# davxy/ark-ec-vrfs

Measured on AMD Instinct MI355X. Metric: Bandersnatch IETF-ECVRF verifies/sec, 2^20 batch per GPU, higher is better.
Workload: dtype u32; 1 GPU; IETF ECVRF verify, Bandersnatch_SHA-512_ELL2, batch 2^20 per GPU, compressed points (161 B/verify), checked decode: on curve + prime-order subgroup, as arkworks' deserialisation, ad="", about 1 in 16 proofs forged (BASELINE.json configs[2]); global_batch=1048576, parallelism=items sharded x1, result gather only, subgroup_check=True

## Files before the change

### ark_ec_vrfs_amd/csrc/fe.cuh

```cuda
#pragma once
#include <hip/hip_runtime.h>
#include <cstdint>
#include "field.h"
#include "vrf_types.h"

VRF_NS_BEGIN

using vrfk::LMASK;
constexpr int NL = 9;
constexpr int LW = 29;

constexpr int mul_v(int v1, int v2) {
  return vrfk::FIELD_KIND == 2 ? 2 : 1 + (v1 * v2 * vrfk::MULV_NUM + 99999) / 100000;
}

template <int L, int V>
struct Fe {
  static_assert(L >= 1 && L <= 7, "limb bound out of range");
  static_assert(V >= 1 && V <= vrfk::VMAX, "value bound out of range (top limb must stay < 2^29)");
  uint32_t v[NL];
  Fe() = default;
  template <int L2, int V2>
  VRF_HD Fe(const Fe<L2, V2>& o) {
    static_assert(L2 <= L && V2 <= V, "narrowing Fe conversion");
#pragma unroll
    for (int i = 0; i < NL; ++i) v[i] = o.v[i];
  }
};

using FeN = Fe<1, 2>;
using FeP = Fe<1, 5>;

template <int L, int V>
VRF_HD Fe<L, V> fe_load(const uint32_t* p) {
  Fe<L, V> r;
#pragma unroll
  for (int i = 0; i < NL; ++i) r.v[i] = p[i];
  return r;
}
VRF_HD FeN fe_const(const uint32_t (&c)[NL]) {
  FeN r;
#pragma unroll
  for (int i = 0; i < NL; ++i) r.v[i] = c[i];
  return r;
}
template <int L, int V>
VRF_HD void fe_store(uint32_t* p, const Fe<L, V>& a) {
#pragma unroll
  for (int i = 0; i < NL; ++i) p[i] = a.v[i];
}

VRF_HD FeN fe_zero() {
  FeN r;
#pragma unroll
  for (int i = 0; i < NL; ++i) r.v[i] = 0;
  return r;
}
VRF_HD FeN fe_one() { return fe_const(vrfk::ONE_M); }

template <int L1, int V1, int L2, int V2>
VRF_HD Fe<L1 + L2, V1 + V2> fe_add(const Fe<L1, V1>& a, const Fe<L2, V2>& b) {
  Fe<L1 + L2, V1 + V2> r;
#pragma unroll
  for (int i = 0; i < NL; ++i) r.v[i] = a.v[i] + b.v[i];
  return r;
}

template <int K, int LB>
struct Bias;
#define VRF_BIAS(K_, LB_)                                            \
  template <>                                                        \
  struct Bias<K_, LB_> {                                             \
    static VRF_HD uint32_t at(int i) { return vrfk::BIAS_L##LB_##_K##K_[i]; } \
  };
VRF_BIAS(4, 1) VRF_BIAS(8, 1) VRF_BIAS(16, 1) VRF_BIAS(32, 1) VRF_BIAS(64, 1)
VRF_BIAS(4, 2) VRF_BIAS(8, 2) VRF_BIAS(16, 2) VRF_BIAS(32, 2) VRF_BIAS(64, 2)
#undef VRF_BIAS

constexpr int bias_k(int v) { return v < 4 ? 4 : v < 8 ? 8 : v < 16 ? 16 : v < 32 ? 32 : 64; }

template <int L1, int V1, int L2, int V2>
VRF_HD Fe<L1 + L2 + 1, V1 + bias_k(V2)> fe_sub(const Fe<L1, V1>& a, const Fe<L2, V2>& b) {
  static_assert(L2 <= 2, "subtrahend must have L <= 2 (normalise first)");
  constexpr int K = bias_k(V2);
  Fe<L1 + L2 + 1, V1 + K> r;
#pragma unroll
  for (int i = 0; i < NL; ++i) r.v[i] = a.v[i] + (Bias<K, L2>::at(i) - b.v[i]);
  return r;
}

template <int L, int V>
VRF_HD Fe<L + 1, bias_k(V)> fe_neg(const Fe<L, V>& b) {
  static_assert(L <= 2, "fe_neg operand must have L <= 2");
  constexpr int K = bias_k(V);
  Fe<L + 1, K> r;
#pragma unroll
  for (int i = 0; i < NL; ++i) r.v[i] = Bias<K, L>::at(i) - b.v[i];
  return r;
}

template <int L, int V>
VRF_HD Fe<2 * L, 2 * V> fe_dbl(const Fe<L, V>& a) {
  Fe<2 * L, 2 * V> r;
#pragma unroll
  for (int i = 0; i < NL; ++i) r.v[i] = a.v[i] << 1;
  return r;
}
template <int L, int V>
VRF_HD Fe<5 * L, 5 * V> fe_mul5(const Fe<L, V>& a) {
  Fe<5 * L, 5 * V> r;
#pragma unroll
  for (int i = 0; i < NL; ++i) r.v[i] = (a.v[i] << 2) + a.v[i];
  return r;
}

template <int L, int V>
VRF_HD Fe<1, V> fe_norm(const Fe<L, V>& a) {
  Fe<1, V> r;
  r.v[0] = a.v[0] & LMASK;
#pragma unroll
  for (int i = 1; i < NL - 1; ++i) r.v[i] = (a.v[i] & LMASK) + (a.v[i - 1] >> LW);
  r.v[NL - 1] = a.v[NL - 1] + (a.v[NL - 2] >> LW);
  return r;
}

#if VRF_FIELD == 3
template <int L, int V>
VRF_HD Fe<1, 2> fe_wred(const Fe<L, V>& a) {
  uint32_t x[NL];
  uint32_t c = 0;
#pragma unroll
  for (int i = 0; i < NL - 1; ++i) {
    const uint32_t t = a.v[i] + c;
    x[i] = t & LMASK;
    c = t >> LW;
  }
  x[NL - 1] = a.v[NL - 1] + c;
  const int32_t k = (int32_t)(x[NL - 1] >> 24);
  x[NL - 1] &= 0x00ffffffu;
  Fe<1, 2> r;
  int32_t cc = k;
#pragma unroll
  for (int i = 0; i < NL; ++i) {
    int32_t t = (int32_t)x[i] + cc;
    if (i == 3) t -= k << 9;
    if (i == 6) t -= k << 18;
    if (i == 7) t += k << 21;
    r.v[i] = (i < NL - 1) ? ((uint32_t)t & LMASK) : (uint32_t)t;
    cc = t >> LW;
  }
  return r;
}
#endif

template <int L, int V>
VRF_HD Fe<L, V> fe_select(bool c, const Fe<L, V>& a, const Fe<L, V>& b) {
  Fe<L, V> r;
#pragma unroll
  for (int i = 0; i < NL; ++i) r.v[i] = c ? a.v[i] : b.v[i];
  return r;
}

VRF_HD uint64_t mad(uint32_t a, uint32_t b, uint64_t c) { return (uint64_t)a * b + c; }
VRF_HD constexpr uint64_t mont_bias() { return vrfk::FIELD_KIND == 0 ? (uint64_t)LMASK : 0; }
VRF_HD uint32_t mont_digit(uint32_t col) {
  if constexpr (vrfk::FIELD_KIND == 0) return ~col & LMASK;
  else return (col * vrfk::NINV29) & LMASK;
}
constexpr uint32_t PM_FOLD = 1216;
constexpr int PM_TOPBITS = 23;

template <int V>
VRF_HD void pm_fold(Fe<1, V>& r, const uint32_t (&d)[2 * NL]) {
  uint64_t acc = 0;
#pragma unroll
  for (int k = 0; k < NL - 1; ++k) {
    acc = mad(d[k + NL], PM_FOLD, acc + d[k]);
    r.v[k] = (uint32_t)acc & LMASK;
    acc >>= LW;
  }
  acc = mad(d[2 * NL - 1], PM_FOLD, acc + d[NL - 1]);
  r.v[NL - 1] = (uint32_t)acc & ((1u << PM_TOPBITS) - 1);
  const uint32_t c = (uint32_t)(acc >> PM_TOPBITS);
  const uint32_t r0 = r.v[0] + 19u * c;
  r.v[0] = r0 & LMASK;
  r.v[1] += r0 >> LW;
}

template <int L1, int V1, int L2, int V2>
VRF_HD Fe<1, mul_v(V1, V2)> fe_mul(const Fe<L1, V1>& a, const Fe<L2, V2>& b) {
  static_assert(L1 * L2 <= 6, "fe_mul: 64-bit column accumulator could overflow");
  Fe<1, mul_v(V1, V2)> r;
  if constexpr (vrfk::FIELD_KIND == 2) {
    uint32_t d[2 * NL];
    uint64_t acc = 0;
#pragma unroll
    for (int k = 0; k < 2 * NL - 1; ++k) {
#pragma unroll
      for (int i = (k < NL ? 0 : k - NL + 1); i <= (k < NL ? k : NL - 1); ++i) acc = mad(a.v[i], b.v[k - i], acc);
      d[k] = (uint32_t)acc & LMASK;
      acc >>= LW;
    }
    d[2 * NL - 1] = (uint32_t)acc;
    pm_fold(r, d);
    return r;
  } else {
  uint32_t m[NL];
  uint64_t acc = 0;
#pragma unroll
  for (int k = 0; k < NL; ++k) {
    acc += mont_bias();
#pragma unroll
    for (int i = 0; i <= k; ++i) acc = mad(a.v[i], b.v[k - i], acc);
#pragma unroll
    for (int i = 0; i < k; ++i) acc = mad(m[i], vrfk::Q29[k - i], acc);
    m[k] = mont_digit((uint32_t)acc);
    if constexpr (vrfk::FIELD_KIND != 0) acc = mad(m[k], vrfk::Q29[0], acc);
    acc >>= LW;
  }
#pragma unroll
  for (int k = NL; k < 2 * NL - 1; ++k) {
#pragma unroll
    for (int i = k - NL + 1; i < NL; ++i) acc = mad(a.v[i], b.v[k - i], acc);
#pragma unroll
    for (int i = k - NL + 1; i < NL; ++i) acc = mad(m[i], vrfk::Q29[k - i], acc);
    r.v[k - NL] = (uint32_t)acc & LMASK;
    acc >>= LW;
  }
  r.v[NL - 1] = (uint32_t)acc;
  return r;
  }
}

template <int L, int V>
VRF_HD Fe<1, mul_v(V, V)> fe_sqr(const Fe<L, V>& a) {
  static_assert(L * L <= 6, "fe_sqr: 64-bit column accumulator could overflow");
  Fe<1, mul_v(V, V)> r;
  uint32_t a2[NL];
#pragma unroll
  for (int i = 0; i < NL; ++i) a2[i] = a.v[i] << 1;
  if constexpr (vrfk::FIELD_KIND == 2) {
    uint32_t d[2 * NL];
    uint64_t acc = 0;
#pragma unroll
    for (int k = 0; k < 2 * NL - 1; ++k) {
#pragma unroll
      for (int i = (k < NL ? 0 : k - NL + 1); 2 * i < k; ++i) acc = mad(a2[i], a.v[k - i], acc);
      if ((k & 1) == 0) acc = mad(a.v[k / 2], a.v[k / 2], acc);
      d[k] = (uint32_t)acc & LMASK;
      acc >>= LW;
    }
    d[2 * NL - 1] = (uint32_t)acc;
    pm_fold(r, d);
    return r;
  } else {
  uint32_t m[NL];
  uint64_t acc = 0;
#pragma unroll
  for (int k = 0; k < NL; ++k) {
    acc += mont_bias();
#pragma unroll
    for (int i = 0; 2 * i < k; ++i) acc = mad(a2[i], a.v[k - i], acc);
    if ((k & 1) == 0) acc = mad(a.v[k / 2], a.v[k / 2], acc);
#pragma unroll
    for (int i = 0; i < k; ++i) acc = mad(m[i], vrfk::Q29[k - i], acc);
    m[k] = mont_digit((uint32_t)acc);
    if constexpr (vrfk::FIELD_KIND != 0) acc = mad(m[k], vrfk::Q29[0], acc);
    acc >>= LW;
  }
#pragma unroll
  for (int k = NL; k < 2 * NL - 1; ++k) {
#pragma unroll
    for (int i = k - NL + 1; 2 * i < k; ++i) acc = mad(a2[i], a.v[k - i], acc);
    if ((k & 1) == 0) acc = mad(a.v[k / 2], a.v[k / 2], acc);
#pragma unroll
    for (int i = k - NL + 1; i < NL; ++i) acc = mad(m[i], vrfk::Q29[k - i], acc);
    r.v[k - NL] = (uint32_t)acc & LMASK;
    acc >>= LW;
  }
  r.v[NL - 1] = (uint32_t)acc;
  return r;
  }
}

template <int L>
VRF_HD void fe_reduce_once(uint32_t out[NL], const Fe<L, 2>& a) {
  uint32_t x[NL], d[NL];
  uint32_t c = 0;
#pragma unroll
  for (int i = 0; i < NL - 1; ++i) {
    uint32_t t = a.v[i] + c;
    x[i] = t & LMASK;
    c = t >> LW;
  }
  x[NL - 1] = a.v[NL - 1] + c;
  uint32_t borrow = 0;
#pragma unroll
  for (int i = 0; i < NL; ++i) {
    uint32_t t = x[i] - vrfk::Q29[i] - borrow;
    borrow = t >> 31;
    d[i] = (i < NL - 1) ? (t & LMASK) : t;
  }
#pragma unroll
  for (int i = 0; i < NL; ++i) out[i] = borrow ? x[i] : d[i];
}

template <int L, int V>
VRF_HD FeN fe_canon(const Fe<L, V>& a) {
  static_assert(L <= 6, "");
  FeN t = fe_mul(a, fe_one());
  FeN r;
  fe_reduce_once(r.v, t);
  return r;
}

template <int L, int V>
VRF_HD bool fe_is_zero(const Fe<L, V>& a) {
  FeN c = fe_canon(a);
  uint32_t o = 0;
#pragma unroll
  for (int i = 0; i < NL; ++i) o |= c.v[i];
  return o == 0;
}

template <int L1, int V1, int L2, int V2>
VRF_HD bool fe_eq(const Fe<L1, V1>& a, const Fe<L2, V2>& b) {
  FeN x = fe_canon(a), y = fe_canon(b);
  uint32_t o = 0;
#pragma unroll
  for (int i = 0; i < NL; ++i) o |= x.v[i] ^ y.v[i];
  return o == 0;
}

VRF_HD void u256_to_limbs(uint32_t out[NL], const uint32_t w[8]) {
#pragma unroll
  for (int i = 0; i < NL; ++i) {
    const int bit = i * LW, j = bit >> 5, s = bit & 31;
    uint32_t lo = w[j] >> s;
    if (s > 3 && j + 1 < 8) lo |= w[j + 1] << (32 - s);
    out[i] = (i < NL - 1) ? (lo & LMASK) : lo;
  }
}
VRF_HD void limbs_to_u256(uint32_t w[8], const uint32_t x[NL]) {
#pragma unroll
  for (int j = 0; j < 8; ++j) {
    const int bit = j * 32, i = bit / LW, s = bit % LW;
    uint32_t v = x[i] >> s;
    if (i + 1 < NL) v |= x[i + 1] << (LW - s);
    if (LW - s + LW < 32 && i + 2 < NL) v |= x[i + 2] << (2 * LW - s);
    w[j] = v;
  }
}

VRF_HD FeN fe_from_u256(const uint32_t w[8]) {
  Fe<1, vrfk::V256> t;
  u256_to_limbs(t.v, w);
  return fe_mul(t, fe_const(vrfk::R2_29));
}
template <int L, int V>
VRF_HD void fe_to_u256(uint32_t w[8], const Fe<L, V>& a) {
  static_assert(L <= 6, "");
  FeN one;
#pragma unroll
  for (int i = 0; i < NL; ++i) one.v[i] = (i == 0);
  FeN t = fe_mul(a, one);
  uint32_t c[NL];
  fe_reduce_once(c, t);
  limbs_to_u256(w, c);
}

VRF_HD FeN fe_from_abi(uint32_t canon[8], const uint32_t w[8], bool mont256) {
  Fe<1, vrfk::V256> t;
  u256_to_limbs(t.v, w);
  FeN k;
#pragma unroll
  for (int i = 0; i < NL; ++i) k.v[i] = mont256 ? vrfk::TWO266_29[i] : vrfk::R2_29[i];
  const FeN r = fe_mul(t, k);
  if (mont256) {
    fe_to_u256(canon, r);
  } else {
#pragma unroll
    for (int i = 0; i < 8; ++i) canon[i] = w[i];
  }
  return r;
}
template <int L, int V>
VRF_HD void fe_to_mont256(uint32_t w[8], const Fe<L, V>& a) {
  static_assert(L <= 6, "");
  FeN t = fe_mul(a, fe_const(vrfk::TWO256_29));
  uint32_t c[NL];
  fe_reduce_once(c, t);
  limbs_to_u256(w, c);
}
VRF_HD void u256_canon_to_mont256(uint32_t w[8]) {
  Fe<1, vrfk::V256> t;
  u256_to_limbs(t.v, w);
  FeN k;
#pragma unroll
  for (int i = 0; i < NL; ++i) k.v[i] = vrfk::R2_29[i];
  fe_to_mont256(w, fe_mul(t, k));
}

VRF_HD Fe<1, 4> fe_from_u512(const uint32_t w[16]) {
  Fe<1, vrfk::V256> lo, hi;
  u256_to_limbs(lo.v, w);
  u256_to_limbs(hi.v, w + 8);
  FeN a = fe_mul(lo, fe_const(vrfk::R2_29));
  FeN b = fe_mul(hi, fe_const(vrfk::TWO256_R2));
  return fe_norm(fe_add(a, b));
}

template <int LEN>
VRF_HD FeN fe_pow_prog(const FeN& x, const uint16_t (&prog)[LEN]) {
  FeN t[8];
  t[0] = x;
  const FeN x2 = fe_sqr(x);
#pragma unroll
  for (int i = 1; i < 8; ++i) t[i] = fe_mul(t[i - 1], x2);
  auto pick = [&](uint32_t idx) {
    FeN s = t[0];
#pragma unroll
    for (int j = 1; j < 8; ++j)
      if (idx == (uint32_t)j) s = t[j];
    return s;
  };
  FeN acc = pick(prog[0] & 15u);
#pragma unroll 1
  for (int i = 1; i < LEN; ++i) {
    const uint32_t op = prog[i], nsq = op >> 4, idx = op & 15u;
#pragma unroll 1
    for (uint32_t k = 0; k < nsq; ++k) acc = fe_sqr(acc);
    if (idx != 15u) acc = fe_mul(acc, pick(idx));
  }
  return acc;
}

template <int L, int V>
VRF_HD FeN fe_inv_pow(const Fe<L, V>& a) {
  FeN x = fe_mul(a, fe_one());
  return fe_pow_prog(x, vrfk::POW_INV_PROG);
}

VRF_HD uint32_t sqrt_lut_index(const SqrtTables& T, const FeN& y) {
  FeN c = fe_canon(y);
  uint32_t h = (c.v[0] * vrfk::SQRT_LUT_MULT) >> (32 - vrfk::SQRT_LUT_BITS);
  return T.lut[h];
}
VRF_HD FeN sqrt_tbl(const SqrtTables& T, int k, uint32_t j) {
  return fe_load<1, 2>(T.P + ((size_t)k * 256 + j) * NL);
}
VRF_HD bool limbs_eq(const FeN& a, const uint32_t (&c)[NL]) {
  uint32_t o = 0;
#pragma unroll
  for (int i = 0; i < NL; ++i) o |= a.v[i] ^ c[i];
  return o == 0;
}

VRF_HD bool sqrt_finish(FeN& root, const FeN& x0, uint32_t e, const SqrtTables& T) {
  bool odd = e & 1;
  uint32_t half = (e >> 1) + (e & 1);
  FeN r = fe_mul(x0, sqrt_tbl(T, 0, half & 255));
  r = fe_mul(r, sqrt_tbl(T, 1, (half >> 8) & 255));
  r = fe_mul(r, sqrt_tbl(T, 2, (half >> 16) & 255));
  r = fe_mul(r, sqrt_tbl(T, 3, half >> 24));
  FeN rz = fe_mul(r, fe_const(vrfk::SQRT_CZ_M));
  root = fe_select(odd, rz, r);
  return !odd;
}

template <int L, int V>
VRF_HD bool fe_sqrt_or_zsqrt(FeN& root, const Fe<L, V>& w_in, const SqrtTables& T) {
  FeN w = fe_mul(w_in, fe_one());
  FeN v = fe_pow_prog(w, vrfk::POW_SQRT_PROG);
  FeN x0 = fe_mul(w, v);
  FeN b = fe_mul(x0, v);
  if constexpr (vrfk::SQRT_S == 1) {
    root = x0;
    const FeN bc = fe_canon(b);
    uint32_t nz = 0;
#pragma unroll
    for (int i = 0; i < NL; ++i) nz |= bc.v[i];
    return limbs_eq(bc, vrfk::ONE_M) || nz == 0;
  } else if constexpr (vrfk::SQRT_S == 2) {
#if VRF_FIELD == 1
    uint32_t e;
    const FeN bc = fe_canon(b);
    e = limbs_eq(bc, vrfk::SQRT_G1_M) ? 1u : limbs_eq(bc, vrfk::SQRT_G2_M) ? 2u : limbs_eq(bc, vrfk::SQRT_G3_M) ? 3u : 0u;
    const bool odd = e & 1;
    const uint32_t half = (e >> 1) + (e & 1);
    const FeN hm = fe_select(half == 0, fe_one(), fe_select(half == 1, fe_const(vrfk::SQRT_H1_M), fe_const(vrfk::SQRT_H2_M)));
    FeN r = fe_mul(x0, hm);
    FeN rz = fe_mul(r, fe_const(vrfk::SQRT_CZ_M));
    root = fe_select(odd, rz, r);
    return !odd;
#endif
  } else if constexpr (vrfk::SQRT_S == 28) {
    FeN b4 = b;
    for (int i = 0; i < 4; ++i) b4 = fe_sqr(b4);
    FeN b12 = b4;
    for (int i = 0; i < 8; ++i) b12 = fe_sqr(b12);
    FeN b20 = b12;
    for (int i = 0; i < 8; ++i) b20 = fe_sqr(b20);
    uint32_t e0 = sqrt_lut_index(T, b20);
    uint32_t e1 = sqrt_lut_index(T, fe_mul(b12, sqrt_tbl(T, 5, e0)));
    uint32_t e2 = sqrt_lut_index(T, fe_mul(fe_mul(b4, sqrt_tbl(T, 4, e0)), sqrt_tbl(T, 5, e1)));
    uint32_t e3 = sqrt_lut_index(
        T, fe_mul(fe_mul(fe_mul(b, sqrt_tbl(T, 0, e0)), sqrt_tbl(T, 1, e1)), sqrt_tbl(T, 2, e2))) >> 4;
    return sqrt_finish(root, x0, e0 | (e1 << 8) | (e2 << 16) | (e3 << 24), T);
  } else {
    static_assert(vrfk::SQRT_S <= 2 || vrfk::SQRT_S == 28 || vrfk::SQRT_S == 32, "no square-root plan for this 2-adicity");
    FeN b8 = b;
    for (int i = 0; i < 8; ++i) b8 = fe_sqr(b8);
    FeN b16 = b8;
    for (int i = 0; i < 8; ++i) b16 = fe_sqr(b16);
    FeN b24 = b16;
    for (int i = 0; i < 8; ++i) b24 = fe_sqr(b24);
    uint32_t e0 = sqrt_lut_index(T, b24);
    uint32_t e1 = sqrt_lut_index(T, fe_mul(b16, sqrt_tbl(T, 2, e0)));
    uint32_t e2 = sqrt_lut_index(T, fe_mul(fe_mul(b8, sqrt_tbl(T, 1, e0)), sqrt_tbl(T, 2, e1)));
    uint32_t e3 = sqrt_lut_index(
        T, fe_mul(fe_mul(fe_mul(b, sqrt_tbl(T, 0, e0)), sqrt_tbl(T, 1, e1)), sqrt_tbl(T, 2, e2)));
    return sqrt_finish(root, x0, e0 | (e1 << 8) | (e2 << 16) | (e3 << 24), T);
  }
}


template <int L, int V>
VRF_HD uint32_t fe_dlog2_low8(const Fe<L, V>& w_in, const SqrtTables& T) {
  static_assert(L > 0 && vrfk::SQRT_S >= 8, "the field has no 2^8-torsion");
  FeN w = fe_mul(w_in, fe_one());
  FeN v = fe_pow_prog(w, vrfk::POW_SQRT_PROG);
  FeN b = fe_mul(fe_mul(w, v), v);
  for (int i = 0; i < vrfk::SQRT_S - 8; ++i) b = fe_sqr(b);
  return sqrt_lut_index(T, b);
}

static_assert(vrfk::CHI_R == 1, "jacobi_limbs callers assume chi(R) = 1");
constexpr int JAC_K = 29;
constexpr int JAC_MAX_ROUNDS = 40;

VRF_HD bool vrf_any(bool x) {
#if defined(__HIP_DEVICE_COMPILE__)
  return __any((int)x) != 0;
#else
  return x;
#endif
}

VRF_HD int jacobi_limbs(const uint32_t x[NL]) {
  uint32_t f[NL], g[NL];
  uint32_t nz = 0, dq = 0;
#pragma unroll
  for (int i = 0; i < NL; ++i) { f[i] = vrfk::Q29[i]; g[i] = x[i]; nz |= x[i]; dq |= x[i] ^ vrfk::Q29[i]; }
  const bool zero = nz == 0 || dq == 0;
  int32_t eta = -1;
  uint32_t jac = 0;
  bool done = zero;
#pragma unroll 1
  for (int round = 0; round < JAC_MAX_ROUNDS; ++round) {
    if (!vrf_any(!done)) break;
    uint32_t f0 = f[0] | (f[1] << LW), g0 = g[0] | (g[1] << LW);
    uint32_t u = 1, v = 0, q = 0, r = 1, jl = jac;
    int32_t e = eta;
#pragma unroll
    for (int i = 0; i < JAC_K; ++i) {
      const uint32_t m = 0u - (g0 & 1u);
      const uint32_t sw = m & (uint32_t)(e >> 31);
      jl ^= f0 & g0 & sw;
      uint32_t t = (f0 ^ g0) & sw; f0 ^= t; g0 ^= t;
      t = (u ^ q) & sw; u ^= t; q ^= t;
      t = (v ^ r) & sw; v ^= t; r ^= t;
      e = (e ^ (int32_t)sw) - (int32_t)sw;
      g0 += f0 & m; q += u & m; r += v & m;
      g0 >>= 1; u <<= 1; v <<= 1; e -= 1;
      jl ^= f0 ^ (f0 >> 1);
    }
    uint32_t nf[NL], ng[NL];
    uint64_t af = mad(u, f[0], (uint64_t)v * g[0]) >> LW, ag = mad(q, f[0], (uint64_t)r * g[0]) >> LW;
#pragma unroll
    for (int i = 1; i < NL; ++i) {
      af = mad(u, f[i], mad(v, g[i], af));
      ag = mad(q, f[i], mad(r, g[i], ag));
      nf[i - 1] = (uint32_t)af & LMASK; af >>= LW;
      ng[i - 1] = (uint32_t)ag & LMASK; ag >>= LW;
    }
    nf[NL - 1] = (uint32_t)af; ng[NL - 1] = (uint32_t)ag;
    uint32_t rest = 0;
#pragma unroll
    for (int i = 1; i < NL; ++i) rest |= nf[i];
    const bool now_one = nf[0] == 1u && rest == 0;
#pragma unroll
    for (int i = 0; i < NL; ++i) { f[i] = done ? f[i] : nf[i]; g[i] = done ? g[i] : ng[i]; }
    eta = done ? eta : e;
    jac = done ? jac : jl;
    done = done || now_one;
  }
  if (zero) return 0;
  if (!done) return 2;
  return (jac & 2u) ? -1 : 1;
}

template <int L, int V>
VRF_HD bool fe_is_nonzero_square(const Fe<L, V>& w, const SqrtTables& T) {
  const FeN c = fe_canon(w);
  const int j = jacobi_limbs(c.v);
  if (j == 2) {
    FeN root;
    return fe_sqrt_or_zsqrt(root, c, T) && !fe_is_zero(c);
  }
  return j == 1;
}

template <int L, int V>
VRF_HD bool fe_is_square_or_zero(const Fe<L, V>& w, const SqrtTables& T) {
  const FeN c = fe_canon(w);
  const int j = jacobi_limbs(c.v);
  if (j == 2) {
    FeN root;
    return fe_sqrt_or_zsqrt(root, c, T) || fe_is_zero(c);
  }
  return j >= 0;
}

template <bool CT = false, int L, int V>
VRF_HD FeN fe_inv(const Fe<L, V>& a) {
  const FeN c = fe_canon(a);
  uint32_t f[NL], g[NL], d[NL], e[NL];
  uint32_t nz = 0;
#pragma unroll
  for (int i = 0; i < NL; ++i) { f[i] = vrfk::Q29[i]; g[i] = c.v[i]; d[i] = 0; e[i] = (i == 0); nz |= c.v[i]; }
  int32_t eta = -1;
  bool done = nz == 0;
#pragma unroll 1
  for (int round = 0; round < JAC_MAX_ROUNDS; ++round) {
    if (!CT && !vrf_any(!done)) break;
    uint32_t f0 = f[0] | (f[1] << LW), g0 = g[0] | (g[1] << LW);
    uint32_t u = 1, v = 0, q = 0, r = 1;
    int32_t et = eta;
#pragma unroll
    for (int i = 0; i < JAC_K; ++i) {
      const uint32_t m = 0u - (g0 & 1u);
      const uint32_t sw = m & (uint32_t)(et >> 31);
      uint32_t t = (f0 ^ g0) & sw; f0 ^= t; g0 ^= t;
      t = (u ^ q) & sw; u ^= t; q ^= t;
      t = (v ^ r) & sw; v ^= t; r ^= t;
      et = (et ^ (int32_t)sw) - (int32_t)sw;
      g0 += f0 & m; q += u & m; r += v & m;
      g0 >>= 1; u <<= 1; v <<= 1; et -= 1;
    }
    uint32_t nf[NL], ng[NL], nd[NL], ne[NL];
    uint64_t af = mad(u, f[0], (uint64_t)v * g[0]) >> LW, ag = mad(q, f[0], (uint64_t)r * g[0]) >> LW;
    const uint64_t td = mad(u, d[0], (uint64_t)v * e[0]), te = mad(q, d[0], (uint64_t)r * e[0]);
    const uint32_t md = ((uint32_t)td * vrfk::NINV29) & LMASK, me = ((uint32_t)te * vrfk::NINV29) & LMASK;
    uint64_t ad = mad(md, vrfk::Q29[0], td) >> LW, ae = mad(me, vrfk::Q29[0], te) >> LW;
#pragma unroll
    for (int i = 1; i < NL; ++i) {
      af = mad(u, f[i], mad(v, g[i], af));
      ag = mad(q, f[i], mad(r, g[i], ag));
      ad = mad(u, d[i], mad(v, e[i], mad(md, vrfk::Q29[i], ad)));
      ae = mad(q, d[i], mad(r, e[i], mad(me, vrfk::Q29[i], ae)));
      nf[i - 1] = (uint32_t)af & LMASK; af >>= LW;
      ng[i - 1] = (uint32_t)ag & LMASK; ag >>= LW;
      nd[i - 1] = (uint32_t)ad & LMASK; ad >>= LW;
      ne[i - 1] = (uint32_t)ae & LMASK; ae >>= LW;
    }
    nf[NL - 1] = (uint32_t)af; ng[NL - 1] = (uint32_t)ag; nd[NL - 1] = (uint32_t)ad; ne[NL - 1] = (uint32_t)ae;
    uint32_t rest = 0;
#pragma unroll
    for (int i = 1; i < NL; ++i) rest |= nf[i];
    const bool now_one = nf[0] == 1u && rest == 0;
#pragma unroll
    for (int i = 0; i < NL; ++i) {
      f[i] = done ? f[i] : nf[i]; g[i] = done ? g[i] : ng[i];
      d[i] = done ? d[i] : nd[i]; e[i] = done ? e[i] : ne[i];
    }
    eta = done ? eta : et;
    done = done || now_one;
  }
  if (vrf_any(!done)) {
    const FeN slow = fe_inv_pow(a);
    if (!done) return slow;
  }
  Fe<(vrfk::VMAX < 64 ? 2 : 1), (vrfk::VMAX < 64 ? vrfk::VMAX : 64)> dd;
#pragma unroll
  for (int i = 0; i < NL; ++i) dd.v[i] = nz == 0 ? 0u : d[i];
  return fe_mul(fe_mul(dd, fe_const(vrfk::R2_29)), fe_const(vrfk::R2_29));
}

VRF_NS_END
```

Baseline: 26.29 million verifies/s.

## Use variable-time batched divsteps with ctz skipping in Jacobi and inversion

Replaces the fixed 29 constant-time divsteps per round in the Jacobi symbol and non-CT inversion with a variable-time loop. It skips runs of zero bits via count-trailing-zeros and eliminates up to 4 bits at a time with a small multiplier lookup formula (Bernstein-Yang / Pornin style). The aim is fewer ALU operations per round. In exchange it adds data-dependent branching, which on a GPU causes divergence within a wavefront, and the jac sign tracking must stay correct under multi-bit steps.

```diff
diff --git a/ark_ec_vrfs_amd/csrc/fe.cuh b/ark_ec_vrfs_amd/csrc/fe.cuh
--- a/ark_ec_vrfs_amd/csrc/fe.cuh
+++ b/ark_ec_vrfs_amd/csrc/fe.cuh
@@ -538,6 +538,7 @@
 static_assert(vrfk::CHI_R == 1, "jacobi_limbs callers assume chi(R) = 1");
 constexpr int JAC_K = 29;
 constexpr int JAC_MAX_ROUNDS = 40;
+static_assert(JAC_K + 3 <= 32, "after JAC_K steps the low words must still hold the bits 1 and 2 that the sign reads");
 
 VRF_HD bool vrf_any(bool x) {
 #if defined(__HIP_DEVICE_COMPILE__)
@@ -545,6 +546,50 @@
 #else
   return x;
 #endif
+}
+
+struct JacTrans { uint32_t u, v, q, r; };
+
+VRF_HD int32_t jac_steps_ct(int32_t eta, uint32_t f, uint32_t g, JacTrans& t) {
+  uint32_t u = 1, v = 0, q = 0, r = 1;
+#pragma unroll
+  for (int i = 0; i < JAC_K; ++i) {
+    const uint32_t m = 0u - (g & 1u);
+    const uint32_t sw = m & (uint32_t)(eta >> 31);
+    uint32_t x = (f ^ g) & sw; f ^= x; g ^= x;
+    x = (u ^ q) & sw; u ^= x; q ^= x;
+    x = (v ^ r) & sw; v ^= x; r ^= x;
+    eta = (eta ^ (int32_t)sw) - (int32_t)sw;
+    g += f & m; q += u & m; r += v & m;
+    g >>= 1; u <<= 1; v <<= 1; eta -= 1;
+  }
+  t = JacTrans{u, v, q, r};
+  return eta;
+}
+
+template <bool SIGN>
+VRF_HD int32_t jac_steps_var(int32_t eta, uint32_t f, uint32_t g, int left, JacTrans& t, uint32_t& jac) {
+  uint32_t u = 1, v = 0, q = 0, r = 1;
+  int i = left;
+#pragma unroll 1
+  for (;;) {
+    const int z = __builtin_ctz(g | (~0u << i));
+    g >>= z; u <<= z; v <<= z; eta -= z; i -= z;
+    if (SIGN) jac ^= (f ^ (f >> 1)) & ((uint32_t)z << 1);
+    if (i == 0) break;
+    const bool sw = eta < 0;
+    if (SIGN) jac ^= sw ? f & g : 0u;
+    const uint32_t nf = sw ? g : f, ng = sw ? f : g, nu = sw ? q : u, nq = sw ? u : q, nv = sw ? r : v, nr = sw ? v : r;
+    f = nf; g = ng; u = nu; q = nq; v = nv; r = nr;
+    eta = sw ? -eta : eta;
+    int k = eta + 1 < i ? eta + 1 : i;
+    k = k < 4 ? k : 4;
+    const uint32_t f4 = f & 15u, g4 = g & 15u;
+    const uint32_t w = (g4 * f4 * ((f4 * f4 + 14u) & 15u)) & ((1u << k) - 1u);
+    g += f * w; q += u * w; r += v * w;
+  }
+  t = JacTrans{u, v, q, r};
+  return eta;
 }
 
 VRF_HD int jacobi_limbs(const uint32_t x[NL]) {
@@ -559,22 +604,11 @@
 #pragma unroll 1
   for (int round = 0; round < JAC_MAX_ROUNDS; ++round) {
     if (!vrf_any(!done)) break;
-    uint32_t f0 = f[0] | (f[1] << LW), g0 = g[0] | (g[1] << LW);
-    uint32_t u = 1, v = 0, q = 0, r = 1, jl = jac;
-    int32_t e = eta;
-#pragma unroll
-    for (int i = 0; i < JAC_K; ++i) {
-      const uint32_t m = 0u - (g0 & 1u);
-      const uint32_t sw = m & (uint32_t)(e >> 31);
-      jl ^= f0 & g0 & sw;
-      uint32_t t = (f0 ^ g0) & sw; f0 ^= t; g0 ^= t;
-      t = (u ^ q) & sw; u ^= t; q ^= t;
-      t = (v ^ r) & sw; v ^= t; r ^= t;
-      e = (e ^ (int32_t)sw) - (int32_t)sw;
-      g0 += f0 & m; q += u & m; r += v & m;
-      g0 >>= 1; u <<= 1; v <<= 1; e -= 1;
-      jl ^= f0 ^ (f0 >> 1);
-    }
+    const uint32_t f0 = f[0] | (f[1] << LW), g0 = g[0] | (g[1] << LW);
+    uint32_t jl = jac;
+    JacTrans t;
+    const int32_t e = jac_steps_var<true>(eta, f0, g0, done ? 0 : JAC_K, t, jl);
+    const uint32_t u = t.u, v = t.v, q = t.q, r = t.r;
     uint32_t nf[NL], ng[NL];
     uint64_t af = mad(u, f[0], (uint64_t)v * g[0]) >> LW, ag = mad(q, f[0], (uint64_t)r * g[0]) >> LW;
 #pragma unroll
@@ -634,20 +668,16 @@
 #pragma unroll 1
   for (int round = 0; round < JAC_MAX_ROUNDS; ++round) {
     if (!CT && !vrf_any(!done)) break;
-    uint32_t f0 = f[0] | (f[1] << LW), g0 = g[0] | (g[1] << LW);
-    uint32_t u = 1, v = 0, q = 0, r = 1;
-    int32_t et = eta;
-#pragma unroll
-    for (int i = 0; i < JAC_K; ++i) {
-      const uint32_t m = 0u - (g0 & 1u);
-      const uint32_t sw = m & (uint32_t)(et >> 31);
-      uint32_t t = (f0 ^ g0) & sw; f0 ^= t; g0 ^= t;
-      t = (u ^ q) & sw; u ^= t; q ^= t;
-      t = (v ^ r) & sw; v ^= t; r ^= t;
-      et = (et ^ (int32_t)sw) - (int32_t)sw;
-      g0 += f0 & m; q += u & m; r += v & m;
-      g0 >>= 1; u <<= 1; v <<= 1; et -= 1;
+    const uint32_t f0 = f[0] | (f[1] << LW), g0 = g[0] | (g[1] << LW);
+    JacTrans t;
+    int32_t et;
+    if constexpr (CT) {
+      et = jac_steps_ct(eta, f0, g0, t);
+    } else {
+      uint32_t no_sign = 0;
+      et = jac_steps_var<false>(eta, f0, g0, done ? 0 : JAC_K, t, no_sign);
     }
+    const uint32_t u = t.u, v = t.v, q = t.q, r = t.r;
     uint32_t nf[NL], ng[NL], nd[NL], ne[NL];
     uint64_t af = mad(u, f[0], (uint64_t)v * g[0]) >> LW, ag = mad(q, f[0], (uint64_t)r * g[0]) >> LW;
     const uint64_t td = mad(u, d[0], (uint64_t)v * e[0]), te = mad(q, d[0], (uint64_t)r * e[0]);
```

New measurement: 27.04 million verifies/s (median of 6 runs). 2.8% higher.
